# WWWindrunner/Cross-Modal-Video-Engine

Hardware: AMD Instinct MI355X
Metric: query-video pairs/sec scored + R@1/5/10 parity, MSR-VTT-1kA at 1/8 GPU (higher is better)
Workload: dtype f16

## Files before the change

cross-modal-video-engine_amd/csrc/cmve_internal.h:

```cpp
#pragma once
#include <hip/hip_runtime.h>
#include <hip/hip_ext.h>
#include <stdint.h>
#include <math.h>
#include <string>
#include <algorithm>
#include <type_traits>
#include "../../include/cmve.h"

struct cmve_handle {
  int device;
  hipStream_t stream;
  hipStream_t aux = nullptr;
  hipEvent_t ev[CMVE_MAX_CHUNKS + 2] = {};
  hipEvent_t tev[2 * CMVE_MAX_CHUNKS] = {};
  int last_chunks = 0;
  hipEvent_t eval_ev[CMVE_EVAL_TIMING_SLOTS][4] = {};
  hipEvent_t eval_kev[CMVE_EVAL_TIMING_SLOTS][8] = {};
  bool eval_no_fix[CMVE_EVAL_TIMING_SLOTS] = {};
  bool eval_chained[CMVE_EVAL_TIMING_SLOTS] = {};
  void* scratch = nullptr;
  size_t scratch_bytes = 0;
  void* comm = nullptr;
  int nranks = 1, rank = 0;
};

namespace cmve {

void set_error(const char* fmt, ...);
int check_launch(const char* what);
int ensure_scratch(cmve_handle* h, size_t bytes);
void dist_release(cmve_handle* h);
int merge_topk_launch(hipStream_t s, const int64_t* ids, const double* scores, int64_t n_q, int lists, int k_in,
                      int64_t q_stride, int64_t l_stride, int k_out, int64_t* out_ids, double* out_scores);
struct LaunchEv {
  hipEvent_t start = nullptr, stop = nullptr;
};
extern thread_local LaunchEv g_launch_ev;
template <typename F, typename... Args>
inline void launch(F kernel, dim3 grid, dim3 block, uint32_t shmem, hipStream_t s, Args... args) {
  if (g_launch_ev.start) {
    const LaunchEv e = g_launch_ev;
    g_launch_ev = LaunchEv{};
    hipExtLaunchKernelGGL(kernel, grid, block, shmem, s, e.start, e.stop, 0u, args...);
  } else {
    hipLaunchKernelGGL(kernel, grid, block, shmem, s, args...);
  }
}
int device_cus();

#define CMVE_REQUIRE(cond, ...)            \
  do {                                     \
    if (!(cond)) {                         \
      ::cmve::set_error(__VA_ARGS__);      \
      return CMVE_E_INVALID;               \
    }                                      \
  } while (0)

#define CMVE_HIP(call)                                                              \
  do {                                                                              \
    hipError_t e_ = (call);                                                         \
    if (e_ != hipSuccess) {                                                         \
      ::cmve::set_error("%s failed: %s", #call, hipGetErrorString(e_));            \
      return CMVE_E_HIP;                                                            \
    }                                                                               \
  } while (0)

constexpr int WAVE = 64;

__device__ __forceinline__ uint16_t f2bf(float f) {
  uint32_t u = __float_as_uint(f);
  if ((u & 0x7fffffffu) > 0x7f800000u) return (uint16_t)((u >> 16) | 0x40u);
  u += 0x7fffu + ((u >> 16) & 1u);
  return (uint16_t)(u >> 16);
}
__device__ __forceinline__ float bf2f(uint16_t b) { return __uint_as_float(((uint32_t)b) << 16); }

__device__ __forceinline__ double wave_sum(double v) {
#pragma unroll
  for (int o = 32; o >= 1; o >>= 1) v += __shfl_xor(v, o, 64);
  return v;
}
__device__ __forceinline__ float wave_max(float v) {
#pragma unroll
  for (int o = 32; o >= 1; o >>= 1) v = fmaxf(v, __shfl_xor(v, o, 64));
  return v;
}
__device__ __forceinline__ int wave_sum_i(int v) {
#pragma unroll
  for (int o = 32; o >= 1; o >>= 1) v += __shfl_xor(v, o, 64);
  return v;
}

#define CMVE_GP(T) __attribute__((address_space(1))) T*
template <typename T> __device__ __forceinline__ T gld(const T* p) { return *(const CMVE_GP(T))p; }
template <typename T, typename U> __device__ __forceinline__ void gst(T* p, U v) { *(CMVE_GP(T))p = (T)v; }
template <typename T> __device__ __forceinline__ T gadd(T* p, T v) {
  return __hip_atomic_fetch_add((CMVE_GP(T))p, v, __ATOMIC_RELAXED, __HIP_MEMORY_SCOPE_AGENT);
}
template <typename T> __device__ __forceinline__ T gmax(T* p, T v) {
  return __hip_atomic_fetch_max((CMVE_GP(T))p, v, __ATOMIC_RELAXED, __HIP_MEMORY_SCOPE_AGENT);
}
template <typename T> __device__ __forceinline__ T gmin(T* p, T v) {
  return __hip_atomic_fetch_min((CMVE_GP(T))p, v, __ATOMIC_RELAXED, __HIP_MEMORY_SCOPE_AGENT);
}

template <typename T> __device__ __forceinline__ double ld64(const T* p) { return (double)gld(p); }

typedef float cmve_f32x4 __attribute__((ext_vector_type(4)));
typedef double cmve_f64x2 __attribute__((ext_vector_type(2)));

__device__ __forceinline__ void load4d(const float* p, double (&v)[4]) {
  const cmve_f32x4 x = gld((const cmve_f32x4*)p);
  v[0] = x.x;
  v[1] = x.y;
  v[2] = x.z;
  v[3] = x.w;
}
__device__ __forceinline__ void load4d(const double* p, double (&v)[4]) {
  const cmve_f64x2 x = gld((const cmve_f64x2*)p), y = gld((const cmve_f64x2*)(p + 2));
  v[0] = x.x;
  v[1] = x.y;
  v[2] = y.x;
  v[3] = y.y;
}
template <typename T>
__host__ __device__ __forceinline__ bool rows_vec4(const T* p, int64_t d, int64_t ld) {
  return (d & 3) == 0 && ((ld * (int64_t)sizeof(T)) & 15) == 0 && (((uintptr_t)p) & 15) == 0;
}

template <typename TA, typename TB, bool LIGHT = false>
__device__ __forceinline__ double wave_dot64(const TA* __restrict__ a, const TB* __restrict__ b,
                                             int64_t d, int lane) {
  double acc = 0.0;
  if ((d & 3) == 0 && ((((uintptr_t)a) | ((uintptr_t)b)) & 15) == 0) {
    auto fma4 = [&](const double (&x)[4], const double (&y)[4]) {
#pragma unroll
      for (int c = 0; c < 4; ++c) acc = fma(x[c], y[c], acc);
    };
    int64_t k = (int64_t)lane * 4;
    for (; k + 768 < d; k += 1024) {
      if constexpr (LIGHT) {
#pragma unroll
        for (int h = 0; h < 2; ++h) {
          double a0[4], a1[4], b0[4], b1[4];
          load4d(a + k + 512 * h, a0);
          load4d(a + k + 512 * h + 256, a1);
          load4d(b + k + 512 * h, b0);
          load4d(b + k + 512 * h + 256, b1);
          fma4(a0, b0);
          fma4(a1, b1);
          __builtin_amdgcn_sched_barrier(0);
        }
        continue;
      }
      double a0[4], a1[4], a2[4], a3[4], b0[4], b1[4], b2[4], b3[4];
      load4d(a + k, a0);
      load4d(a + k + 256, a1);
      load4d(a + k + 512, a2);
      load4d(a + k + 768, a3);
      load4d(b + k, b0);
      load4d(b + k + 256, b1);
      load4d(b + k + 512, b2);
      load4d(b + k + 768, b3);
      fma4(a0, b0);
      fma4(a1, b1);
      fma4(a2, b2);
      fma4(a3, b3);
    }
    {
      double x[3][4], y[3][4];
#pragma unroll
      for (int m = 0; m < 3; ++m)
        if (k + 256 * m < d) {
          load4d(a + k + 256 * m, x[m]);
          load4d(b + k + 256 * m, y[m]);
        }
#pragma unroll
      for (int m = 0; m < 3; ++m)
        if (k + 256 * m < d) fma4(x[m], y[m]);
    }
    return wave_sum(acc);
  }
  for (int64_t k = lane; k < d; k += WAVE) acc = fma(ld64(a + k), ld64(b + k), acc);
  return wave_sum(acc);
}

template <typename TA, typename TB>
__device__ __forceinline__ void wave_dot64_x2(const TA* __restrict__ a, const TB* __restrict__ b,
                                              const TA* __restrict__ a2, const TB* __restrict__ b2, int64_t d,
                                              int lane, double& s1, double& s2) {
  if ((d & 3) == 0 && ((((uintptr_t)a) | ((uintptr_t)b) | ((uintptr_t)a2) | ((uintptr_t)b2)) & 15) == 0) {
    double acc = 0.0, acc2 = 0.0;
    auto fma4 = [](double& s, const double (&x)[4], const double (&y)[4]) {
#pragma unroll
      for (int c = 0; c < 4; ++c) s = fma(x[c], y[c], s);
    };
    int64_t k = (int64_t)lane * 4;
    for (; k + 768 < d; k += 1024) {
      double x[4][4], y[4][4], x2[4][4], y2[4][4];
#pragma unroll
      for (int m = 0; m < 4; ++m) {
        load4d(a + k + 256 * m, x[m]);
        load4d(b + k + 256 * m, y[m]);
        load4d(a2 + k + 256 * m, x2[m]);
        load4d(b2 + k + 256 * m, y2[m]);
      }
#pragma unroll
      for (int m = 0; m < 4; ++m) {
        fma4(acc, x[m], y[m]);
        fma4(acc2, x2[m], y2[m]);
      }
    }
    for (; k < d; k += 256) {
      double x[4], y[4], x2[4], y2[4];
      load4d(a + k, x);
      load4d(b + k, y);
      load4d(a2 + k, x2);
      load4d(b2 + k, y2);
      fma4(acc, x, y);
      fma4(acc2, x2, y2);
    }
#pragma unroll
    for (int o = 32; o >= 1; o >>= 1) {
      acc += __shfl_xor(acc, o, 64);
      acc2 += __shfl_xor(acc2, o, 64);
    }
    s1 = acc;
    s2 = acc2;
    return;
  }
  s1 = wave_dot64(a, b, d, lane);
  s2 = wave_dot64(a2, b2, d, lane);
}

__device__ __forceinline__ float f32_round_up(double x) {
  float f = (float)x;
  if ((double)f < x) f = nextafterf(f, INFINITY);
  return f;
}
__device__ __forceinline__ float f32_round_down(double x) {
  float f = (float)x;
  if ((double)f > x) f = nextafterf(f, -INFINITY);
  return f;
}

template <typename T>
__device__ __forceinline__ double row_sumsq(const T* __restrict__ x, int64_t d, bool vec, int lane) {
  double ss = 0.0;
  if (vec) {
    for (int64_t k = (int64_t)lane * 4; k < d; k += 256) {
      double v[4];
      load4d(x + k, v);
#pragma unroll
      for (int c = 0; c < 4; ++c) ss = fma(v[c], v[c], ss);
    }
    return wave_sum(ss);
  }
  for (int64_t k = lane; k < d; k += WAVE) {
    const double v = (double)x[k];
    ss = fma(v, v, ss);
  }
  return wave_sum(ss);
}
__device__ __forceinline__ double row_inv_norm(double ss, double eps, int flags) {
  const double nrm = sqrt(ss);
  return (flags & CMVE_PACK_RAW) ? 1.0 : (eps > 0.0 ? 1.0 / fmax(nrm, eps) : 1.0 / nrm);
}

struct PackAcc {
  double e1 = 0.0, e2 = 0.0, e3 = 0.0;
  float e4 = 0.f;
};

__device__ __forceinline__ int xcd_linear(int bid, int total) {
  const int xcd = bid & 7, local = bid >> 3;
  const int q = total >> 3, r = total & 7;
  return (xcd < r ? xcd * (q + 1) : r * (q + 1) + (xcd - r) * q) + local;
}

__device__ __forceinline__ uint32_t lo8_scale_bits(float hf) {
  return max(__float_as_uint(hf) & 0x7f800000u, 113u << 23) - (18u << 23);
}
__device__ __forceinline__ float lo8_elem(float xf, float hf, float& res) {
  const uint32_t sb = lo8_scale_bits(hf);
  const float d2 = xf - hf;
  const float q = __builtin_amdgcn_fmed3f(__builtin_rintf(d2 * __uint_as_float((254u << 23) - sb)), -128.f, 127.f);
  res = fmaf(-q, __uint_as_float(sb), d2);
  return q;
}
__device__ __forceinline__ uint32_t lo8_put(uint32_t w, int c, float q) {
  return __builtin_amdgcn_cvt_pk_u8_f32(q + 128.f, (uint32_t)c, w);
}
constexpr uint32_t LO8_ZERO4 = 0x80808080u;
__device__ __forceinline__ float lo8_bound(double ss_res) {
  return f32_round_up(sqrt(ss_res) * (1.0 + 1e-4) + 5.9605e-8 * (1.0 + 1e-6) + 1e-12);
}
__device__ __forceinline__ _Float16 f16_via_f32(double xh, float& xf) {
  xf = (float)xh;
  asm volatile("" : "+v"(xf));
  return (_Float16)xf;
}

__device__ __forceinline__ void pack_elem(double xh, bool want_f16, uint16_t& h, uint16_t& l, uint16_t& f,
                                          PackAcc& acc) {
  float xf;
  const _Float16 hf16 = f16_via_f32(xh, xf);
  if (want_f16) {
    const double r3 = xh - (double)hf16;
    acc.e3 = fma(r3, r3, acc.e3);
    f = __builtin_bit_cast(uint16_t, hf16);
  }
  h = f2bf(xf);
  const float hf = bf2f(h);
  l = f2bf(xf - hf);
  const double r1 = xh - (double)hf;
  const double r2 = r1 - (double)bf2f(l);
  acc.e1 = fma(r1, r1, acc.e1);
  acc.e2 = fma(r2, r2, acc.e2);
}

typedef unsigned short cmve_u16x4 __attribute__((ext_vector_type(4)));
typedef uint32_t cmve_u32x2 __attribute__((ext_vector_type(2)));

__device__ __forceinline__ void pack_pad_row(uint16_t* hrow, uint16_t* lrow, uint16_t* frow, int64_t d_pad,
                                             int lane) {
  const cmve_u16x4 z = {0, 0, 0, 0};
  for (int64_t k = (int64_t)lane * 4; k < d_pad; k += 256) {
    gst((cmve_u16x4*)(hrow + k), z);
    if (lrow) gst((cmve_u16x4*)(lrow + k), z);
    if (frow) gst((cmve_u16x4*)(frow + k), z);
  }
}

template <typename T>
__device__ __forceinline__ void pack_row_planes(const T* __restrict__ x, int64_t d, int64_t d_pad, bool vec,
                                                double inv, uint16_t* hrow, uint16_t* lrow, uint16_t* frow,
                                                int lane, float& b1, float& b2, float& b3) {
  const bool want_f16 = frow != nullptr;
  PackAcc acc;
  bool done = false;
  if (vec) {
    for (int64_t k = (int64_t)lane * 4; k < d_pad; k += 256) {
      cmve_u16x4 hv = {0, 0, 0, 0}, lv = {0, 0, 0, 0}, fv = {0, 0, 0, 0};
      if (k < d) {
        double e[4];
        load4d(x + k, e);
#pragma unroll
        for (int c = 0; c < 4; ++c) {
          uint16_t h, l, f = 0;
          pack_elem(e[c] * inv, want_f16, h, l, f, acc);
          hv[c] = h;
          lv[c] = l;
          fv[c] = f;
        }
      }
      *(cmve_u16x4*)(hrow + k) = hv;
      if (lrow) *(cmve_u16x4*)(lrow + k) = lv;
      if (frow) *(cmve_u16x4*)(frow + k) = fv;
    }
    done = true;
  }
  if (!done)
    for (int64_t k = lane; k < d_pad; k += WAVE) {
      uint16_t h = 0, l = 0, f = 0;
      if (k < d) pack_elem((double)x[k] * inv, want_f16, h, l, f, acc);
      hrow[k] = h;
      if (lrow) lrow[k] = l;
      if (frow) frow[k] = f;
    }
  const double e1 = wave_sum(acc.e1), e2 = wave_sum(acc.e2), e3 = wave_sum(acc.e3);
  b1 = f32_round_up(sqrt(e1) * (1.0 + 1e-9) + 1e-12);
  b2 = f32_round_up(sqrt(e2) * (1.0 + 1e-9) + 1e-12);
  b3 = f32_round_up(sqrt(e3) * (1.0 + 1e-9) + 1e-12);
}

__device__ __forceinline__ int64_t gt_rank_of(int32_t cnt, double sgt, int64_t n_m) {
  return (sgt != sgt) ? n_m + 1 : (sgt == (double)INFINITY ? n_m : (int64_t)cnt + 1);
}

constexpr int CAND_BUCKET_SHIFT = 8;
struct CandLayout {
  int64_t nb, cap_b;
};
inline CandLayout cand_layout(int64_t g_n_pad, int64_t cap) {
  CandLayout l;
  l.nb = std::max<int64_t>(1, (g_n_pad + (1 << CAND_BUCKET_SHIFT) - 1) >> CAND_BUCKET_SHIFT);
  l.cap_b = cap > l.nb ? (cap - l.nb) / l.nb : 0;
  return l;
}
constexpr int64_t FIXUP_MAX_BUCKETS_PER_XCD = 4096;
constexpr int EVAL_EMAX_SHARDS = 64;

template <typename TA, typename TB, bool LIGHT = false>
__device__ __forceinline__ double wave_cos64(const TA* xa, const TB* xb, double inva, double invb, int64_t d,
                                             int lane) {
  return wave_dot64<TA, TB, LIGHT>(xa, xb, d, lane) * (inva * invb);
}

typedef uint32_t cmve_u32x4 __attribute__((ext_vector_type(4)));
struct L16Frag {
  cmve_u32x4 h0, h1, r;
};
__device__ __forceinline__ void l16_load(const uint16_t* __restrict__ hrow, const uint8_t* __restrict__ rrow,
                                         int64_t k, L16Frag& f) {
  f.h0 = gld((const cmve_u32x4*)(hrow + k));
  f.h1 = gld((const cmve_u32x4*)(hrow + k + 8));
  f.r = gld((const cmve_u32x4*)(rrow + k));
}
template <int E>
__device__ __forceinline__ double l16_x(uint32_t hw, uint32_t rw) {
  const float hf = (float)__builtin_bit_cast(_Float16, (uint16_t)(hw >> (16 * (E & 1))));
  const float sc = __uint_as_float(lo8_scale_bits(hf));
  const float u = (float)((rw >> (8 * (E & 3))) & 0xffu);
  return (double)fmaf(u, sc, fmaf(-128.f, sc, hf));
}
__device__ __forceinline__ double l16_partial(const L16Frag& a, const L16Frag& b) {
  const uint32_t ah[8] = {a.h0.x, a.h0.y, a.h0.z, a.h0.w, a.h1.x, a.h1.y, a.h1.z, a.h1.w};
  const uint32_t ar[4] = {a.r.x, a.r.y, a.r.z, a.r.w};
  const uint32_t bh[8] = {b.h0.x, b.h0.y, b.h0.z, b.h0.w, b.h1.x, b.h1.y, b.h1.z, b.h1.w};
  const uint32_t br[4] = {b.r.x, b.r.y, b.r.z, b.r.w};
  double acc0 = 0.0, acc1 = 0.0;
#pragma unroll
  for (int w = 0; w < 8; w += 2) {
    acc0 = fma(l16_x<0>(ah[w], ar[w / 2]), l16_x<0>(bh[w], br[w / 2]), acc0);
    acc1 = fma(l16_x<1>(ah[w], ar[w / 2]), l16_x<1>(bh[w], br[w / 2]), acc1);
    acc0 = fma(l16_x<2>(ah[w + 1], ar[w / 2]), l16_x<2>(bh[w + 1], br[w / 2]), acc0);
    acc1 = fma(l16_x<3>(ah[w + 1], ar[w / 2]), l16_x<3>(bh[w + 1], br[w / 2]), acc1);
  }
  return acc0 + acc1;
}
template <int CTRL>
__device__ __forceinline__ double l16_dpp(double v) {
  const uint64_t b = __builtin_bit_cast(uint64_t, v);
  const uint32_t lo = (uint32_t)__builtin_amdgcn_update_dpp(0, (int)(uint32_t)b, CTRL, 0xF, 0xF, false);
  const uint32_t hi = (uint32_t)__builtin_amdgcn_update_dpp(0, (int)(uint32_t)(b >> 32), CTRL, 0xF, 0xF, false);
  return __builtin_bit_cast(double, (uint64_t)lo | ((uint64_t)hi << 32));
}
__device__ __forceinline__ double l16_wave_sum(double v) {
  v += l16_dpp<0xB1>(v);
  v += l16_dpp<0x4E>(v);
  v += l16_dpp<0x141>(v);
  v += l16_dpp<0x140>(v);
  {
    const uint64_t b = __builtin_bit_cast(uint64_t, v);
    const uint32_t lo = (uint32_t)b, hi = (uint32_t)(b >> 32);
    const auto sl = __builtin_amdgcn_permlane16_swap(lo, lo, false, false);
    const auto sh = __builtin_amdgcn_permlane16_swap(hi, hi, false, false);
    v = __builtin_bit_cast(double, (uint64_t)sl[0] | ((uint64_t)sh[0] << 32)) +
        __builtin_bit_cast(double, (uint64_t)sl[1] | ((uint64_t)sh[1] << 32));
  }
  {
    const uint64_t b = __builtin_bit_cast(uint64_t, v);
    const uint32_t lo = (uint32_t)b, hi = (uint32_t)(b >> 32);
    const auto sl = __builtin_amdgcn_permlane32_swap(lo, lo, false, false);
    const auto sh = __builtin_amdgcn_permlane32_swap(hi, hi, false, false);
    v = __builtin_bit_cast(double, (uint64_t)sl[0] | ((uint64_t)sh[0] << 32)) +
        __builtin_bit_cast(double, (uint64_t)sl[1] | ((uint64_t)sh[1] << 32));
  }
  return v;
}
__device__ __forceinline__ void fixup_prefix(const uint64_t* __restrict__ cand, int64_t nb, int64_t cap_b, int xcd,
                                             int G, int64_t nk, int lane, int64_t* pre) {
  const int64_t per = (nk + 63) / 64;
  const int64_t k0 = lane * per, k1 = min(nk, k0 + per);
  if (per <= 4) {
    int64_t v[4];
#pragma unroll
    for (int j = 0; j < 4; ++j) v[j] = (k0 + j < k1) ? min((int64_t)gld(cand + xcd + G * (k0 + j)), cap_b) : 0;
    const int64_t sum = (v[0] + v[1]) + (v[2] + v[3]);
    int64_t incl = sum;
    for (int o = 1; o < 64; o <<= 1) {
      const int64_t t = __shfl_up(incl, o, 64);
      if (lane >= o) incl += t;
    }
    int64_t run = incl - sum;
#pragma unroll
    for (int j = 0; j < 4; ++j)
      if (k0 + j < k1) {
        pre[k0 + j] = run;
        run += v[j];
      }
    if (lane == 63) pre[nk] = incl;
  } else {
    int64_t sum = 0;
    for (int64_t k = k0; k < k1; ++k) sum += min((int64_t)gld(cand + xcd + G * k), cap_b);
    int64_t incl = sum;
    for (int o = 1; o < 64; o <<= 1) {
      const int64_t t = __shfl_up(incl, o, 64);
      if (lane >= o) incl += t;
    }
    int64_t run = incl - sum;
    for (int64_t k = k0; k < k1; ++k) {
      pre[k] = run;
      run += min((int64_t)gld(cand + xcd + G * k), cap_b);
    }
    if (lane == 63) pre[nk] = incl;
  }
}

template <typename TQ, typename TG, bool PREFETCH = false, bool DYN_PRE = false, bool LIGHT = false>
__device__ __forceinline__ void fixup_walk(const TQ* __restrict__ qraw, int64_t ldq,
                                                    const double* __restrict__ qinv, const TG* __restrict__ graw,
                                                    int64_t ldg, const double* __restrict__ ginv, int64_t d,
                                                    const double* __restrict__ row_sgt,
                                                    const double* __restrict__ col_sgt, int* __restrict__ row_cnt,
                                                    int* __restrict__ col_cnt, const uint64_t* __restrict__ cand,
                                                    int64_t nb, int64_t cap_b, bool flat = false) {
  int64_t* pre;
  if constexpr (DYN_PRE) {
    extern __shared__ int64_t fix_dyn_pre[];
    pre = fix_dyn_pre;
  } else {
    __shared__ int64_t fix_pre[FIXUP_MAX_BUCKETS_PER_XCD + 1];
    pre = fix_pre;
  }
  const int lane = threadIdx.x & 63, wave = threadIdx.x >> 6;
  const int G = flat ? 1 : 8;
  const int xcd = flat ? 0 : (blockIdx.x & 7);
  const int64_t nk = xcd < nb ? (nb - xcd + G - 1) / G : 0;
  if (wave == 0) fixup_prefix(cand, nb, cap_b, xcd, G, nk, lane, pre);
  __syncthreads();
  const int64_t total = pre[nk];
  const int nw = (int)(blockDim.x >> 6);
  const int64_t stride = (int64_t)(gridDim.x / G) * nw;
  int64_t k = 0;
  auto entry = [&](int64_t cc) -> uint64_t {
    if (cc >= total) return 0ull;
    if (pre[k + 1] <= cc) {
      int64_t lo = k + 1, hi = nk - 1;
      while (lo < hi) {
        const int64_t mid = (lo + hi + 1) >> 1;
        if (pre[mid] <= cc) lo = mid;
        else hi = mid - 1;
      }
      k = lo;
    }
    return gld(cand + nb + (xcd + G * k) * cap_b + (cc - pre[k]));
  };
  const int64_t c0 = (int64_t)(blockIdx.x / G) * nw + wave;
  uint64_t u_next = entry(c0);
  for (int64_t c = c0; c < total;) {
    const uint64_t u = u_next;
    c += stride;
    u_next = entry(c);
    const int64_t i = (int64_t)(u & 0x7fffffffull);
    const int64_t j = (int64_t)((u >> 31) & 0x7fffffffull);
    uint32_t flags = (uint32_t)(u >> 62);
    if (!flags) continue;
    double rs = 0.0, cs = 0.0;
    if (PREFETCH) {
      rs = ((flags & 1u) && row_sgt) ? gld(row_sgt + i) : 0.0;
      cs = ((flags & 2u) && col_sgt) ? gld(col_sgt + j) : 0.0;
    }
    const double s = wave_cos64<TQ, TG, LIGHT>(qraw + i * ldq, graw + j * ldg, gld(qinv + i), gld(ginv + j), d, lane);
    if (lane == 0) {
      if ((flags & 1u) && row_sgt && s > (PREFETCH ? rs : gld(row_sgt + i))) gadd(row_cnt + i, 1);
      if ((flags & 2u) && col_sgt && s > (PREFETCH ? cs : gld(col_sgt + j))) gadd(col_cnt + j, 1);
    }
  }
}

__device__ __forceinline__ uint32_t topk_key(float f) {
  const uint32_t u = __float_as_uint(f);
  if (f != f) return 0u;
  return (u & 0x80000000u) ? ~u : (u | 0x80000000u);
}
__device__ __forceinline__ float topk_key_inv(uint32_t k) {
  return __uint_as_float((k & 0x80000000u) ? (k & 0x7fffffffu) : ~k);
}

__host__ __device__ __forceinline__ double score_error_bound(double ea, double eb, int64_t d_pad, int mode) {
  const double n = (double)d_pad * (33.0 / 32.0) * (mode == CMVE_SIM_BF16X3 ? 3.0 : 1.0);
  const double u = 1.0 / 8388608.0;
  const double gamma = n * u / (1.0 - n * u);
  return ea + (1.0 + ea) * eb + gamma * (1.0 + ea) * (1.0 + eb) + 1e-12;
}

inline const float* mode_err(const cmve_rows_t* r, int mode) {
  return mode == CMVE_SIM_BF16 ? r->err_hi : (mode == CMVE_SIM_BF16X3 ? r->err_hilo : r->err_h16);
}
__host__ __device__ __forceinline__ int mode_slot(int mode) { return mode; }

}
```

Before: 145.7 billion.

## Encode lo8 residual as integer ULP step on f32 bits instead of scaled float

Replaces the exponent-derived scale quantization of the low-8-bit residual with an integer offset in f32 bit space (step of 32 ULP around the f16 head). The encoder becomes integer add, shift and clamp, and the decoder in the L16 dot-product inner loop becomes a sign-extend plus a shift-add on the head bits, replacing a float scale computation and two FMAs. This changes the numeric representation of the residual, so the error bounds and parity of stored packs depend on the new encoding matching the prior accuracy guarantees. A shared header allows host and device to use the same encode/decode.

```diff
diff --git a/cross-modal-video-engine_amd/csrc/cmve_internal.h b/cross-modal-video-engine_amd/csrc/cmve_internal.h
--- a/cross-modal-video-engine_amd/csrc/cmve_internal.h
+++ b/cross-modal-video-engine_amd/csrc/cmve_internal.h
@@ -7,6 +7,7 @@
 #include <algorithm>
 #include <type_traits>
 #include "../../include/cmve.h"
+#include "lo8_step.h"
 
 struct cmve_handle {
   int device;
@@ -279,19 +280,13 @@
   return (xcd < r ? xcd * (q + 1) : r * (q + 1) + (xcd - r) * q) + local;
 }
 
-__device__ __forceinline__ uint32_t lo8_scale_bits(float hf) {
-  return max(__float_as_uint(hf) & 0x7f800000u, 113u << 23) - (18u << 23);
-}
-__device__ __forceinline__ float lo8_elem(float xf, float hf, float& res) {
-  const uint32_t sb = lo8_scale_bits(hf);
-  const float d2 = xf - hf;
-  const float q = __builtin_amdgcn_fmed3f(__builtin_rintf(d2 * __uint_as_float((254u << 23) - sb)), -128.f, 127.f);
-  res = fmaf(-q, __uint_as_float(sb), d2);
-  return q;
-}
-__device__ __forceinline__ uint32_t lo8_put(uint32_t w, int c, float q) {
-  return __builtin_amdgcn_cvt_pk_u8_f32(q + 128.f, (uint32_t)c, w);
-}
+__device__ __forceinline__ uint32_t lo8_elem(float xf, float hf, float& res) {
+  const uint32_t B = __float_as_uint(hf);
+  const uint32_t u = lo8_step_encode(__float_as_uint(xf), B);
+  res = xf - __uint_as_float(lo8_step_decode(B, u));
+  return u;
+}
+__device__ __forceinline__ uint32_t lo8_put(uint32_t w, int c, uint32_t u) { return w | (u << (8 * c)); }
 constexpr uint32_t LO8_ZERO4 = 0x80808080u;
 __device__ __forceinline__ float lo8_bound(double ss_res) {
   return f32_round_up(sqrt(ss_res) * (1.0 + 1e-4) + 5.9605e-8 * (1.0 + 1e-6) + 1e-12);
@@ -409,24 +404,26 @@
   f.r = gld((const cmve_u32x4*)(rrow + k));
 }
 template <int E>
-__device__ __forceinline__ double l16_x(uint32_t hw, uint32_t rw) {
+__device__ __forceinline__ double l16_x(uint32_t hw, uint32_t rs, int sh) {
   const float hf = (float)__builtin_bit_cast(_Float16, (uint16_t)(hw >> (16 * (E & 1))));
-  const float sc = __uint_as_float(lo8_scale_bits(hf));
-  const float u = (float)((rw >> (8 * (E & 3))) & 0xffu);
-  return (double)fmaf(u, sc, fmaf(-128.f, sc, hf));
+  const int32_t q = (int32_t)(rs << (24 - 8 * (E & 3))) >> 24;
+  return (double)__uint_as_float(lo8_step_decode_q(__float_as_uint(hf), q, sh));
 }
 __device__ __forceinline__ double l16_partial(const L16Frag& a, const L16Frag& b) {
   const uint32_t ah[8] = {a.h0.x, a.h0.y, a.h0.z, a.h0.w, a.h1.x, a.h1.y, a.h1.z, a.h1.w};
-  const uint32_t ar[4] = {a.r.x, a.r.y, a.r.z, a.r.w};
+  constexpr uint32_t S = 0x80808080u;
+  const uint32_t ar[4] = {a.r.x ^ S, a.r.y ^ S, a.r.z ^ S, a.r.w ^ S};
   const uint32_t bh[8] = {b.h0.x, b.h0.y, b.h0.z, b.h0.w, b.h1.x, b.h1.y, b.h1.z, b.h1.w};
-  const uint32_t br[4] = {b.r.x, b.r.y, b.r.z, b.r.w};
+  const uint32_t br[4] = {b.r.x ^ S, b.r.y ^ S, b.r.z ^ S, b.r.w ^ S};
+  int sh = 5;
+  asm("" : "+s"(sh));
   double acc0 = 0.0, acc1 = 0.0;
 #pragma unroll
   for (int w = 0; w < 8; w += 2) {
-    acc0 = fma(l16_x<0>(ah[w], ar[w / 2]), l16_x<0>(bh[w], br[w / 2]), acc0);
-    acc1 = fma(l16_x<1>(ah[w], ar[w / 2]), l16_x<1>(bh[w], br[w / 2]), acc1);
-    acc0 = fma(l16_x<2>(ah[w + 1], ar[w / 2]), l16_x<2>(bh[w + 1], br[w / 2]), acc0);
-    acc1 = fma(l16_x<3>(ah[w + 1], ar[w / 2]), l16_x<3>(bh[w + 1], br[w / 2]), acc1);
+    acc0 = fma(l16_x<0>(ah[w], ar[w / 2], sh), l16_x<0>(bh[w], br[w / 2], sh), acc0);
+    acc1 = fma(l16_x<1>(ah[w], ar[w / 2], sh), l16_x<1>(bh[w], br[w / 2], sh), acc1);
+    acc0 = fma(l16_x<2>(ah[w + 1], ar[w / 2], sh), l16_x<2>(bh[w + 1], br[w / 2], sh), acc0);
+    acc1 = fma(l16_x<3>(ah[w + 1], ar[w / 2], sh), l16_x<3>(bh[w + 1], br[w / 2], sh), acc1);
   }
   return acc0 + acc1;
 }
diff --git a/cross-modal-video-engine_amd/csrc/lo8_step.h b/cross-modal-video-engine_amd/csrc/lo8_step.h
--- /dev/null
+++ b/cross-modal-video-engine_amd/csrc/lo8_step.h
@@ -0,0 +1,16 @@
+#pragma once
+#include <stdint.h>
+
+#if defined(__HIPCC__) || defined(__CUDACC__)
+#define LO8_STEP_FN __host__ __device__ inline
+#else
+#define LO8_STEP_FN inline
+#endif
+
+LO8_STEP_FN uint32_t lo8_step_encode(uint32_t X, uint32_t B) {
+  const int32_t v = ((int32_t)(X - B) + (4096 + 16)) >> 5;
+  const uint32_t u = (uint32_t)(v < 0 ? 0 : (v > 255 ? 255 : v));
+  return ((B << 1) - 1u >= 0xfeffffffu) ? 128u : u;
+}
+LO8_STEP_FN uint32_t lo8_step_decode(uint32_t B, uint32_t u) { return B - 4096u + (u << 5); }
+LO8_STEP_FN uint32_t lo8_step_decode_q(uint32_t B, int32_t q, int sh = 5) { return B + ((uint32_t)q << sh); }
```

After: 148.1 billion, median of 6. 1.02x the previous value.
